# ZechengLi19/CIM

Measured on AMD Instinct MI355X. Metric: images/sec training step (ResNet-50 VOC, ~1k proposals/img) at 1/2/4/8 GPU, higher is better.
Workload: dtype fp32

## Files before the change

### cim_amd/csrc/gemm_pair.hip

```cpp
#include "common.h"
#include <type_traits>
#include "../../include/cim_hip.h"

namespace {

using f32x16 = __attribute__((ext_vector_type(16))) float;
using f16x8 = __attribute__((ext_vector_type(8))) _Float16;
typedef short s16x4 __attribute__((__vector_size__(4 * sizeof(short))));
typedef short s16x8 __attribute__((__vector_size__(8 * sizeof(short))));

#ifndef CIM_PAIR_EXP
#define CIM_PAIR_EXP 0
#endif
static_assert(CIM_PAIR_EXP == 0 || (CIM_PAIR_EXP >= 3 && CIM_PAIR_EXP <= 5), "CIM_PAIR_EXP: 0 (product), 3, 4 or 5");
constexpr bool ABL_NO_LOOP_DMA = CIM_PAIR_EXP == 3 || CIM_PAIR_EXP == 5;
constexpr bool ABL_NO_LOOP_READS = CIM_PAIR_EXP == 4 || CIM_PAIR_EXP == 5;

constexpr int BM = 256, BN = 256, BK = 32;
constexpr int NW = 8, NT = 64 * NW;
constexpr int WNC = 4;
constexpr int WM = 128, WN = BN / WNC, MI = 4, NI = WN / 32;
constexpr int IPW = 32 / NW;
constexpr int OPER = 256 * BK * 4;
constexpr int SLAB = 2 * OPER;
constexpr int LDS_BYTES = 2 * SLAB;
constexpr int RBM = 128, RBK = 16, RNT = 256, RSTAGES = 5;
constexpr int RSTAGE_A = RBM * RBK * 4, RSTAGE_B = BN * RBK * 4, RSTAGE = RSTAGE_A + RSTAGE_B;
constexpr int RIPA = RSTAGE_A / 1024 / 4, RIPB = RSTAGE_B / 1024 / 4;
constexpr int RLDS_BYTES = RSTAGES * RSTAGE;

enum { L_KC = 0, L_MC = 1 };

struct PairArgs {
    const char* A;
    const char* B;
    float* C;
    const float* bias;
    int M, N, K;
    int lda, ldb, ldc;
    int relu;
    int k_per_split;
    long long c_split_stride;
    int batch;
    long long a_bs, b_bs, c_bs;
    const float* a_scale;
    const float* b_scale;
    unsigned* c_amax;
    int tn, tm, tz;
    int tile0;
// ... 235 lines not shown
template <class Loop>
__device__ __forceinline__ void for_valid_subtiles(int rows, Loop&& loop) {
    switch (__builtin_amdgcn_readfirstlane(min(MI, (rows + 31) / 32))) {
        case 1: loop(std::integral_constant<int, 1>{}); break;
        case 2: loop(std::integral_constant<int, 2>{}); break;
        case 3: loop(std::integral_constant<int, 3>{}); break;
        default: loop(std::integral_constant<int, MI>{}); break;
    }
}

template <int MIV>
struct PairFrags {
    f16x8 ah[MIV > 0 ? MIV : 1], al[MIV > 0 ? MIV : 1], bh[NI], bl[NI];
};

template <int MIV>
__device__ __forceinline__ void mma_cluster(f32x16 (&acc)[MI][NI], const f16x8 (&af)[MIV], const f16x8 (&bf)[NI]) {
#pragma unroll
    for (int i = 0; i < MIV; ++i)
#pragma unroll
        for (int j = 0; j < NI; ++j) acc[i][j] = __builtin_amdgcn_mfma_f32_32x32x16_f16(af[i], bf[j], acc[i][j], 0, 0, 0);
}

template <int NMFMA, int NREAD>
__device__ __forceinline__ void interleave_mfma_reads() {
#pragma unroll
    for (int q = 0; q < NMFMA; ++q) {
        __builtin_amdgcn_sched_group_barrier(0x008, 1, 0);
        if (q < NREAD) __builtin_amdgcn_sched_group_barrier(0x100, 1, 0);
    }
    if constexpr (NREAD > NMFMA) __builtin_amdgcn_sched_group_barrier(0x100, NREAD - NMFMA, 0);
    __builtin_amdgcn_sched_barrier(0);
}

template <int TBM, int SLABK>
__device__ __forceinline__ void pair_epilogue(const PairArgs& g, const PairTile<TBM, SLABK>& T, f32x16 (&acc)[MI][NI], float (&bvj)[NI],
                                              int wm, int wn, int lane) {
    const float inv = 1.0f / (g.a_scale[T.zb] * g.b_scale[T.zb]);
#pragma unroll
    for (int j = 0; j < NI; ++j) asm volatile("" : "+v"(bvj[j]));
    float* C = T.C + (size_t)T.zsplit * g.c_split_stride;
    const int m0 = T.m0, n0 = T.n0;
    const int lk = lane >> 5, l31 = lane & 31;
    unsigned amax = 0;
    const bool relu = g.relu != 0;
    if (m0 + TBM <= g.M && n0 + BN <= g.N) {
#pragma unroll
        for (int j = 0; j < NI; ++j) {
            float* cj = C + (size_t)(m0 + wm * WM + 4 * lk) * g.ldc + n0 + wn * WN + j * 32 + l31;
#pragma unroll
            for (int i = 0; i < MI; ++i) {
#pragma unroll
                for (int r = 0; r < 16; ++r) {
                    float v = acc[i][j][r] * inv + bvj[j];
                    if (relu) v = fmaxf(v, 0.0f);
                    amax = max(amax, abs_bits(v));
                    cj[(size_t)(i * 32 + (r & 3) + 8 * (r >> 2)) * g.ldc] = v;
                }
            }
        }
    } else {
#pragma unroll
        for (int j = 0; j < NI; ++j) {
            const int n = n0 + wn * WN + j * 32 + l31;
            if (n >= g.N) continue;
#pragma unroll
            for (int i = 0; i < MI; ++i) {
#pragma unroll
                for (int r = 0; r < 16; ++r) {
                    const int m = m0 + wm * WM + i * 32 + (r & 3) + 8 * (r >> 2) + 4 * lk;
                    if (m >= g.M) continue;
                    float v = acc[i][j][r] * inv + bvj[j];
                    if (relu) v = fmaxf(v, 0.0f);
                    amax = max(amax, abs_bits(v));
                    C[(size_t)m * g.ldc + n] = v;
                }
            }
        }
    }
    if (g.c_amax != nullptr && g.c_split_stride == 0) {
        amax = wave_max_u32(amax);
        if (lane == 0) cim::amax_publish(g.c_amax, amax);
    }
}

template <int AL, int BL, bool ONEP>
__global__ __launch_bounds__(NT, NW / 4) void gemm_pair_kernel(const PairArgs g) {
    extern __shared__ __attribute__((aligned(16))) char smem[];
    const int tid = threadIdx.x;
    const int wave = __builtin_amdgcn_readfirstlane(tid >> 6), lane = tid & 63;
// ... 37 lines not shown
        constexpr std::bool_constant<(MIV > 0 || AL == L_MC)> with_a{};
        PairFrags<MIV> f0, f1;
        auto read = [&](PairFrags<MIV>& f, const char* buf, int ks, auto in_loop) __attribute__((always_inline)) {
            if constexpr (MIV == 0) {
            } else if constexpr (ABL_NO_LOOP_READS && decltype(in_loop)::value) {
                asm volatile("" : "+v"(f.ah[0]), "+v"(f.al[0]), "+v"(f.bh[0]), "+v"(f.bl[0]));
            } else {
#pragma unroll
                for (int j = 0; j < NI; ++j) {
                    f.bh[j] = fb.read(buf + OPER, j, ks, 0);
                    if constexpr (!ONEP) f.bl[j] = fb.read(buf + OPER, j, ks, 1);
                }
#pragma unroll
                for (int i = 0; i < MIV; ++i) {
                    if constexpr (!ONEP) f.al[i] = fa.read(buf, i, ks, 1);
                    f.ah[i] = fa.read(buf, i, ks, 0);
                }
            }
        };
        auto multiply = [&](const PairFrags<MIV>& f) __attribute__((always_inline)) {
            if constexpr (MIV > 0) {
                if constexpr (AL == L_KC && BL == L_KC) __builtin_amdgcn_sched_barrier(0);
                if constexpr (!ONEP) {
                    mma_cluster(acc, f.al, f.bh);
                    mma_cluster(acc, f.ah, f.bl);
                }
                mma_cluster(acc, f.ah, f.bh);
                if constexpr (AL == L_KC && BL == L_KC) __builtin_amdgcn_sched_barrier(0);
            }
        };
        constexpr std::true_type in_loop{};
        read(f0, smem, 0, std::false_type{});
        if constexpr (ABL_NO_LOOP_READS) read(f1, smem, 1, std::false_type{});
        for (int t = 0; t < nslab; ++t) {
            const char* cur = smem + (t & 1) * SLAB;
            const char* nxt = smem + ((t + 1) & 1) * SLAB;
            read(f1, cur, 1, in_loop);
            multiply(f0);
            asm volatile("s_waitcnt vmcnt(0)" ::: "memory");
            __syncthreads();
            if constexpr (!ABL_NO_LOOP_DMA) {
                if (t + 2 < nslab) issue_slab(cur, with_a);
            }
            if (t + 1 < nslab) read(f0, nxt, 0, in_loop);
            multiply(f1);
        }
    };
    if (wm == 1 && T.m0 + WM >= g.M) {
        prologue(std::bool_constant<AL == L_MC>{});
        slab_loop(std::integral_constant<int, 0>{});
        return;
    }
    prologue(std::true_type{});
    for_valid_subtiles(g.M - T.m0 - wm * WM, slab_loop);

    pair_epilogue(g, T, acc, bvj, wm, wn, lane);
}

template <bool ONEP>
__global__ __launch_bounds__(RNT, 2) void gemm_pair_ring_kernel(const PairArgs g) {
    extern __shared__ __attribute__((aligned(16))) char smem[];
    const int tid = threadIdx.x;
    const int wave = __builtin_amdgcn_readfirstlane(tid >> 6), lane = tid & 63;
    const int wn = wave;
    const PairTile<RBM, RBK> T(g);
    const int nslab = T.nslab;
// ... 390 lines not shown
```

### cim_amd/csrc/roi_align.hip

```cpp
#include <cstdlib>
#include "common.h"
#include "wino7_tile.h"
#include "../../include/cim_hip.h"

namespace {

struct RoiGeom {
    float x1, y1, bw, bh, count;
    int gw, gh, b;
};

#pragma clang fp contract(off)
__device__ __forceinline__ RoiGeom roi_geom(const float* __restrict__ roi, float scale, int P, int sampling_ratio,
                                            int aligned) {
    RoiGeom g;
    const float off = aligned ? 0.5f : 0.0f;
    g.b = (int)roi[0];
    g.x1 = roi[1] * scale - off;
    g.y1 = roi[2] * scale - off;
    const float x2 = roi[3] * scale - off;
    const float y2 = roi[4] * scale - off;
    float rw = x2 - g.x1, rh = y2 - g.y1;
    if (!aligned) {
        rw = fmaxf(rw, 1.0f);
// ... 457 lines not shown
        rs_column_walk(s_rows, s_wa, s_wb, nrows, R.ncols, R.xlo, C, R.fb + c, s_wx, al, ah, bl, bh);
        typedef float ga_f4 __attribute__((ext_vector_type(4)));
#pragma unroll
        for (int pw = 0; pw < 7; ++pw) {
            if (pw >= P) break;
            float* dst = out + (((size_t)k * P + ph0) * P + pw) * OC + c;
            __builtin_nontemporal_store(ga_f4{al[pw].x, al[pw].y, ah[pw].x, ah[pw].y}, reinterpret_cast<ga_f4*>(dst));
            if (MASKCAT) {
                const float m = masks[((size_t)k * P + ph0) * P + pw];
                __builtin_nontemporal_store(ga_f4{m * al[pw].x, m * al[pw].y, m * ah[pw].x, m * ah[pw].y}, reinterpret_cast<ga_f4*>(dst + C));
            }
            if (two) {
                float* dst2 = dst + (size_t)P * OC;
                __builtin_nontemporal_store(ga_f4{bl[pw].x, bl[pw].y, bh[pw].x, bh[pw].y}, reinterpret_cast<ga_f4*>(dst2));
                if (MASKCAT) {
                    const float m = masks[((size_t)k * P + ph0 + 1) * P + pw];
                    __builtin_nontemporal_store(ga_f4{m * bl[pw].x, m * bl[pw].y, m * bh[pw].x, m * bh[pw].y}, reinterpret_cast<ga_f4*>(dst2 + C));
                }
            }
        }
    }
}

__global__ __launch_bounds__(256) void roi_align_wino7_pair_kernel(const float* __restrict__ feat, const float* __restrict__ masks,
                                                                   float* __restrict__ V, int C, int H, int W, int K, int Rs,
                                                                   const float* __restrict__ rec_all,
                                                                   const float* __restrict__ scale) {
    constexpr int P = 7;
    __shared__ __attribute__((aligned(16))) float4 s_patch[49 * 64];
    __shared__ __attribute__((aligned(16))) float s_wx[RS_MAXD][8];
    __shared__ float s_wa[4][RS_MAXD], s_wb[4][RS_MAXD];
    __shared__ int s_rows[4][RS_MAXD];
    __shared__ float s_mask[49];
    const int r = blockIdx.x, slice = blockIdx.y, tid = threadIdx.x, lane = tid & 63, wave = tid >> 6;
    const int c = slice * 256 + lane * 4;
    const size_t C2 = 2 * (size_t)C, MC = (size_t)Rs * C2;
    if (r >= K) {
        if (c < C)
            for (int q = wave; q < 121; q += 4) {
                float* dst = V + (size_t)q * MC + (size_t)r * C2 + c;
                __builtin_nontemporal_store(w7_u4{0, 0, 0, 0}, reinterpret_cast<w7_u4*>(dst));
                __builtin_nontemporal_store(w7_u4{0, 0, 0, 0}, reinterpret_cast<w7_u4*>(dst + C));
            }
        return;
    }
    const int k = r;
    const RoiRec R = roi_rec(rec_all, feat, k, C, H, W, P);
    const int ph0 = wave * 2;
    const bool two = ph0 + 1 < P;
    const int nrows = rs_row_list(R, ph0, two, H, W, lane, s_rows[wave], s_wa[wave], s_wb[wave]);
    rs_fill_wx(s_wx, R, P, W, tid, 256);
    if (tid < 49) s_mask[tid] = masks[(size_t)k * 49 + tid];
    __syncthreads();
    if (c < C) {
        ga_f2 al[7], ah[7], bl[7], bh[7];
        rs_column_walk(s_rows[wave], s_wa[wave], s_wb[wave], nrows, R.ncols, R.xlo, C, R.fb + c, s_wx, al, ah, bl, bh);
#pragma unroll
        for (int pw = 0; pw < 7; ++pw) {
            s_patch[(ph0 * P + pw) * 64 + lane] = make_float4(al[pw].x, al[pw].y, ah[pw].x, ah[pw].y);
            if (two) s_patch[((ph0 + 1) * P + pw) * 64 + lane] = make_float4(bl[pw].x, bl[pw].y, bh[pw].x, bh[pw].y);
        }
    }
    __syncthreads();
    if (c >= C) return;
    const size_t off = (size_t)r * C2 + c;
    const auto plain = [&](int iy, int ix) { return s_patch[(iy * P + ix) * 64 + lane]; };
    const auto masked = [&](int iy, int ix) { return vmul(s_mask[iy * P + ix], s_patch[(iy * P + ix) * 64 + lane]); };
// ... 465 lines not shown

extern "C" int cim_roi_align_bwd_ws(const float* grad_out, const float* rois, float* grad_in, int B, int C, int H, int W,
                                    int K, int P, float spatial_scale, int sampling_ratio, int aligned, float* workspace,
                                    int tables_ready, float* scratch, void* stream) {
    return run_bwd<false>(__func__, grad_out, rois, nullptr, grad_in, B, C, H, W, K, P, spatial_scale, sampling_ratio, aligned, workspace,
                          tables_ready, scratch, stream);
}

extern "C" int cim_roi_align_maskcat_bwd(const float* grad_cat, const float* rois, const float* masks, float* grad_in,
                                         int B, int C, int H, int W, int K, int P, float spatial_scale,
                                         int sampling_ratio, int aligned, float* workspace, void* stream) {
    return run_bwd<true>(__func__, grad_cat, rois, masks, grad_in, B, C, H, W, K, P, spatial_scale, sampling_ratio, aligned, workspace,
                         0, nullptr, stream);
}

extern "C" int cim_roi_align_maskcat_bwd_ws(const float* grad_cat, const float* rois, const float* masks, float* grad_in,
                                            int B, int C, int H, int W, int K, int P, float spatial_scale,
                                            int sampling_ratio, int aligned, float* workspace, int tables_ready,
                                            float* scratch, void* stream) {
    return run_bwd<true>(__func__, grad_cat, rois, masks, grad_in, B, C, H, W, K, P, spatial_scale, sampling_ratio, aligned, workspace,
                         tables_ready, scratch, stream);
}
#undef ROI_CHECK_ARG

extern "C" int cim_roi_align_wino7_pair_fwd(const float* feat, const float* rois, const float* masks, void* V, const float* scale,
                                           int B, int C, int H, int W, int K, int Rs, int P, float spatial_scale,
                                           int sampling_ratio, int aligned, float* workspace, void* stream) {
    CIM_CHECK_ARG(feat && rois && masks && V && scale && workspace);
    CIM_CHECK_ARG(B > 0 && C > 0 && C % 8 == 0 && H > 0 && W > 0 && K > 0 && Rs >= K && P == 7);
    CIM_CHECK_ARG(H <= RS_MAXD && W <= RS_MAXD && (long long)H * W * C < (1ll << 30));
    hipStream_t st = cim::as_stream(stream);
    hipLaunchKernelGGL(roi_tables_kernel, dim3(K), dim3(256), sizeof(float) * roi_rec_words(P, H, W), st, rois, workspace, K, P, H, W,
                       spatial_scale, sampling_ratio, aligned);
    hipLaunchKernelGGL(roi_align_wino7_pair_kernel, dim3((unsigned)Rs, (unsigned)((C + 255) / 256)), dim3(256), 0, st, feat, masks,
                       (float*)V, C, H, W, K, Rs, workspace, scale);
    CIM_CHECK_LAUNCH();
    return 0;
}

extern "C" int cim_roi_align_forms(int B, int C, int H, int W, int K, int P, int maskcat, int has_workspace, int tables_ready,
                                   int* fwd_form, int* bwd_form, int* bwd_builds_tables) {
    CIM_CHECK_ARG(B > 0 && C > 0 && H > 0 && W > 0 && K >= 0 && P > 0 && P <= 65535);
    CIM_CHECK_ARG(fwd_form && bwd_form && bwd_builds_tables && (has_workspace || !tables_ready));
    const RoiForms f = roi_forms(B, C, H, W, K, P, maskcat != 0, has_workspace != 0, tables_ready != 0);
    *fwd_form = f.fwd;
    *bwd_form = f.bwd;
    *bwd_builds_tables = f.bwd_builds_tables ? 1 : 0;
    return 0;
}

extern "C" long long cim_roi_align_bwd_workspace(int K, int P, int H, int W) {
    return (long long)sizeof(float) * (long long)K * roi_rec_words(P, H, W);
}

extern "C" long long cim_roi_align_bwd_scratch(int K, int B, int C, int H, int W) {
    const int GS = rg_group_size(K, B, C, H, W);
    const long long groups = (K + GS - 1) / GS;
    return groups > 1 ? (long long)sizeof(float) * groups * B * H * W * C : 0;
}
```

### cim_amd/csrc/winograd.hip

```cpp
#include "common.h"
#include "../../include/cim_hip.h"
#include "wino7_tile.h"

namespace {

__device__ __forceinline__ float4 f4(float v) { return make_float4(v, v, v, v); }
__device__ __forceinline__ void fma2(float2& a, float s, float2 v) { a.x = fmaf(s, v.x, a.x); a.y = fmaf(s, v.y, a.y); }

typedef float w7_v2 __attribute__((ext_vector_type(2)));
typedef float w7_v4 __attribute__((ext_vector_type(4)));

constexpr int W7_VOUT = 4;
constexpr int W7_VDX = 2;
constexpr int W7_VMF = 1;
constexpr int W7_MF_WAVES = 1;
constexpr int W7_FB_WAVES = 3;
constexpr int W7_WG_CI = 4;

template <int N> struct w7_vec;
template <> struct w7_vec<1> { typedef float T; };
template <> struct w7_vec<2> { typedef float2 T; };
template <> struct w7_vec<4> { typedef float4 T; };
__device__ __forceinline__ void w7_store(float* p, float v) { __builtin_nontemporal_store(v, p); }
__device__ __forceinline__ void w7_store(float* p, float2 v) { __builtin_nontemporal_store(w7_v2{v.x, v.y}, reinterpret_cast<w7_v2*>(p)); }
__device__ __forceinline__ void w7_store(float* p, float4 v) {
    __builtin_nontemporal_store(w7_v4{v.x, v.y, v.z, v.w}, reinterpret_cast<w7_v4*>(p));
}
__device__ __forceinline__ void vzero(float& a) { a = 0.0f; }
__device__ __forceinline__ void vzero(float2& a) { a = make_float2(0.f, 0.f); }
__device__ __forceinline__ void vzero(float4& a) { a = make_float4(0.f, 0.f, 0.f, 0.f); }
__device__ __forceinline__ void vfma(float& a, float s, float v) { a = fmaf(s, v, a); }
__device__ __forceinline__ void vfma(float2& a, float s, float2 v) { fma2(a, s, v); }
__device__ __forceinline__ void vfma(float4& a, float s, float4 v) { fma4(a, s, v); }
__device__ __forceinline__ float vamax(float4 v) { return fmaxf(fmaxf(fabsf(v.x), fabsf(v.y)), fmaxf(fabsf(v.z), fabsf(v.w))); }
__device__ __forceinline__ void vrelu(float4& v) { v = make_float4(fmaxf(v.x, 0.f), fmaxf(v.y, 0.f), fmaxf(v.z, 0.f), fmaxf(v.w, 0.f)); }
template <typename T> __device__ __forceinline__ T vload(const float* p) { return *reinterpret_cast<const T*>(p); }
template <typename T> __device__ __forceinline__ T vload_once(const float* p) {
    if constexpr (sizeof(T) == 4) return __builtin_nontemporal_load(p);
    else if constexpr (sizeof(T) == 8) { const w7_v2 v = __builtin_nontemporal_load(reinterpret_cast<const w7_v2*>(p)); return make_float2(v.x, v.y); }
    else { const w7_v4 v = __builtin_nontemporal_load(reinterpret_cast<const w7_v4*>(p)); return make_float4(v.x, v.y, v.z, v.w); }
}

__device__ __forceinline__ void w7_zero_rows(float* __restrict__ V, int q0, int nq, int r, int Rs, int C) {
    for (int q = q0; q < q0 + nq; ++q)
        for (int c = threadIdx.x * 4; c < C; c += 1024)
            *reinterpret_cast<float4*>(V + ((size_t)q * Rs + r) * C + c) = make_float4(0.f, 0.f, 0.f, 0.f);
}

__global__ __launch_bounds__(256) void wino7_input_pair_kernel(const float* __restrict__ x, float* __restrict__ V, int R, int Rs,
// ... 153 lines not shown
        for (int c = threadIdx.x * 4; c < C; c += 256 * 4) {
            float4 d[OA][OB];
#pragma unroll
            for (int a = 0; a < OA; ++a)
#pragma unroll
                for (int b = 0; b < OB; ++b)
                    d[a][b] = vload<float4>(dy + (((size_t)r * 7 + W7::OUT0[KA] + a) * 7 + W7::OUT0[KB] + b) * C + c);
            w7_dy_tile_regs<KA, KB, ADJ>(d, D, (size_t)Rs * C, (size_t)r * C + c, scale);
        }
    });
}

constexpr int W7_FB_LDW = 260;

template <int KA, int KB, bool ADJ>
__device__ __forceinline__ void w7_fb_tile(const float* __restrict__ s, int lane, float* __restrict__ img, size_t MC, size_t rc,
                                           const float* __restrict__ scale) {
    constexpr int OA = W7::OUT[KA], OB = W7::OUT[KB];
    float4 d[OA][OB];
#pragma unroll
    for (int a = 0; a < OA; ++a)
#pragma unroll
        for (int b = 0; b < OB; ++b)
            d[a][b] = *reinterpret_cast<const float4*>(s + ((W7::OUT0[KA] + a) * 7 + W7::OUT0[KB] + b) * W7_FB_LDW + 4 * lane);
    if (img != nullptr) w7_dy_tile_regs<KA, KB, ADJ>(d, img, MC, rc, scale);
}

__global__ __launch_bounds__(256, W7_FB_WAVES) void wino7_flatten_bwd_dy_pair_kernel(const float* __restrict__ dX, const float* __restrict__ y,
                                                                        float* __restrict__ E, float* __restrict__ D,
                                                                        float* __restrict__ bsum, int R, int Rs, int C,
                                                                        const float* __restrict__ sE, const float* __restrict__ sD) {
    __shared__ __attribute__((aligned(16))) float s[49 * W7_FB_LDW];
    __shared__ float4 red[3][64];
    const int r = blockIdx.x, c0 = blockIdx.y * 256, tid = threadIdx.x, lane = tid & 63;
    const int w = __builtin_amdgcn_readfirstlane(tid >> 6);
    const size_t MC = (size_t)Rs * C, rc = (size_t)r * C + c0 + 4 * lane;
    if (r >= R) {
        const w7_u4 z = {0u, 0u, 0u, 0u};
        for (int q = w; q < 121; q += 4) {
            if (E != nullptr) __builtin_nontemporal_store(z, reinterpret_cast<w7_u4*>(E + (size_t)q * MC + rc));
            if (D != nullptr) __builtin_nontemporal_store(z, reinterpret_cast<w7_u4*>(D + (size_t)q * MC + rc));
        }
        return;
    }
    const float4* __restrict__ src4 = reinterpret_cast<const float4*>(dX + ((size_t)r * C + c0) * 49);
    for (int i = tid; i < 49 * 64; i += 256) {
        const float4 v = vload_once<float4>(reinterpret_cast<const float*>(src4 + i));
        int c = (4 * i) / 49, p = 4 * i - 49 * c;
        const float e[4] = {v.x, v.y, v.z, v.w};
#pragma unroll
        for (int k = 0; k < 4; ++k) {
            s[p * W7_FB_LDW + c] = e[k];
            if (++p == 49) { p = 0; ++c; }
        }
    }
    __syncthreads();
    float4 part = f4(0.f);
    for (int p = w; p < 49; p += 4) {
        float4* sp = reinterpret_cast<float4*>(s + p * W7_FB_LDW + 4 * lane);
        float4 d = *sp;
        if (y != nullptr) {
            const float4 yv = *reinterpret_cast<const float4*>(y + ((size_t)r * 49 + p) * C + c0 + 4 * lane);
            d.x = yv.x > 0.0f ? d.x : 0.0f;
            d.y = yv.y > 0.0f ? d.y : 0.0f;
            d.z = yv.z > 0.0f ? d.z : 0.0f;
            d.w = yv.w > 0.0f ? d.w : 0.0f;
            *sp = d;
        }
        part.x += d.x; part.y += d.y; part.z += d.z; part.w += d.w;
    }
    if (bsum != nullptr && w > 0) red[w - 1][lane] = part;
    __syncthreads();
    if (bsum != nullptr && w == 0) {
        const float4 a = part, b = red[0][lane], c = red[1][lane], e = red[2][lane];
        *reinterpret_cast<float4*>(bsum + rc) = make_float4((a.x + b.x) + (c.x + e.x), (a.y + b.y) + (c.y + e.y),
                                                            (a.z + b.z) + (c.z + e.z), (a.w + b.w) + (c.w + e.w));
    }
    w7_for_tile(w, [&](auto t) __attribute__((always_inline)) {
        w7_fb_tile<t.KA, t.KB, true>(s, lane, E, MC, rc, sE);
        w7_fb_tile<1 - t.KA, 1 - t.KB, false>(s, lane, D, MC, rc, sD);
    });
}

__global__ void wino7_pair_scales_kernel(const unsigned* __restrict__ amax, int n_amax, const unsigned* __restrict__ amax_mul, int kind,
                                         float* __restrict__ scale) {
    const int q = threadIdx.x;
    if (q >= 121) return;
    unsigned mbits = 0;
    for (int t = 0; t < n_amax; ++t) mbits = max(mbits, amax[t] & 0x7fffffffu);
    float dmax = __uint_as_float(mbits);
    if (amax_mul != nullptr) dmax *= fmaxf(1.0f, __uint_as_float(amax_mul[0] & 0x7fffffffu));
    const int type = q < 36 ? 0 : q < 66 ? 1 : q < 96 ? 2 : 3;
    const int ka = type >> 1, kb = type & 1, nb = kb ? 5 : 6, pl = q - W7::QOFF[type];
    const int pi = pl / nb, pj = pl % nb;
    float fa = 0.0f, fb = 0.0f;
    if (kind == 0) {
        for (int t = 0; t < 6; ++t) { fa += fabsf(W7_BT[ka][pi][t]); fb += fabsf(W7_BT[kb][pj][t]); }
    } else if (kind == 1) {
        for (int t = 0; t < 3; ++t) { fa += fabsf(W7_G[ka][pi][t]); fb += fabsf(W7_G[kb][pj][t]); }
    } else if (kind == 2) {
        for (int t = 0; t < 4; ++t) { fa += fabsf(W7_GD[ka][pi][t]); fb += fabsf(W7_GD[kb][pj][t]); }
    } else {
// ... 24 lines not shown
        }
#pragma unroll
        for (int l = 0; l < NB; ++l) {
            const int xx = W7::IN0[KB] + l;
            if (xx < 0 || xx >= P) continue;
#pragma unroll
            for (int j = 0; j < NB; ++j)
                if (W7_BT[KB][j][l] != 0.0f) vfma(acc[yy][xx], W7_BT[KB][j][l], t[j]);
        }
    }
}

__global__ __launch_bounds__(256) void wino7_dx_kernel(const float* __restrict__ M, float* __restrict__ dx, int R, int C) {
    constexpr int VW = W7_VDX;
    typedef typename w7_vec<VW>::T VT;
    const int r = blockIdx.x;
    const size_t MC = (size_t)R * C;
    for (int c = (blockIdx.y * 256 + threadIdx.x) * VW; c < C; c += gridDim.y * 256 * VW) {
        VT acc[7][7];
#pragma unroll
        for (int y = 0; y < 7; ++y)
#pragma unroll
            for (int x = 0; x < 7; ++x) vzero(acc[y][x]);
        const size_t rc = (size_t)r * C + c;
        w7_for_all_tiles([&](auto t) __attribute__((always_inline)) { w7_dx_tile<t.KA, t.KB, VT>(M, MC, rc, acc); });
#pragma unroll
        for (int y = 0; y < 7; ++y)
#pragma unroll
            for (int x = 0; x < 7; ++x) w7_store(dx + (((size_t)r * 7 + y) * 7 + x) * C + c, acc[y][x]);
    }
}

__global__ __launch_bounds__(256, W7_MF_WAVES) void wino7_dx_maskfold_kernel(const float* __restrict__ M, const float* __restrict__ masks,
                                                                float* __restrict__ dbox, int R, int Cb) {
    constexpr int VW = W7_VMF;
    typedef typename w7_vec<VW>::T VT;
    const int r = blockIdx.x;
    const size_t C2 = 2 * (size_t)Cb, MC = (size_t)R * C2;
    const float* __restrict__ mk = masks + (size_t)r * 49;
    for (int c = (blockIdx.y * 256 + threadIdx.x) * VW; c < Cb; c += gridDim.y * 256 * VW) {
        VT acc[7][7];
#pragma unroll
        for (int y = 0; y < 7; ++y)
#pragma unroll
            for (int x = 0; x < 7; ++x) vzero(acc[y][x]);
        const size_t rc = (size_t)r * C2 + c;
        w7_for_all_tiles([&](auto t) __attribute__((always_inline)) { w7_dx_tile<t.KA, t.KB, VT>(M, MC, rc + Cb, acc); });
#pragma unroll
        for (int y = 0; y < 7; ++y)
#pragma unroll
            for (int x = 0; x < 7; ++x) {
                const float m = mk[y * 7 + x];
                VT z;
                vzero(z);
                vfma(z, m, acc[y][x]);
                acc[y][x] = z;
            }
        w7_for_all_tiles([&](auto t) __attribute__((always_inline)) { w7_dx_tile<t.KA, t.KB, VT>(M, MC, rc, acc); });
#pragma unroll
        for (int y = 0; y < 7; ++y)
#pragma unroll
            for (int x = 0; x < 7; ++x) w7_store(dbox + (((size_t)r * 7 + y) * 7 + x) * Cb + c, acc[y][x]);
    }
}

template <int KA, int KB, typename VT>
__device__ __forceinline__ void w7_wgrad_tile(const float* __restrict__ dU, size_t KN, size_t idx, VT (&acc)[3][3]) {
    constexpr int NA = W7::NP[KA], NB = W7::NP[KB], Q0 = W7::QOFF[KA * 2 + KB];
    VT s[3][NB];
#pragma unroll
    for (int a = 0; a < 3; ++a)
#pragma unroll
        for (int j = 0; j < NB; ++j) vzero(s[a][j]);
// ... 57 lines not shown
        const int row = e / ROW, col = e - row * ROW;
        dW[((size_t)(co0 + row) * Cin + ci0) * 9 + col] = t[row][col];
    }
}

__global__ __launch_bounds__(256) void flatten_chw_bwd_kernel(const float* __restrict__ src, const float* __restrict__ y,
                                                              float* __restrict__ dst, int PP, int C, float* __restrict__ bsum) {
    __shared__ float t[64][65];
    const int r = blockIdx.x, c0 = blockIdx.y * 64, tid = threadIdx.x;
    const size_t base = (size_t)r * PP * C;
    for (int e = tid; e < PP * 64; e += 256) {
        const int c = e / PP, p = e - c * PP;
        t[p][c] = src[base + (size_t)c0 * PP + e];
    }
    __syncthreads();
    float part = 0.0f;
    for (int e = tid; e < PP * 64; e += 256) {
        const int p = e >> 6, c = e & 63;
        const size_t o = base + (size_t)p * C + c0 + c;
        const float v = (y == nullptr || y[o] > 0.0f) ? t[p][c] : 0.0f;
        dst[o] = v;
        part += v;
    }
    if (bsum != nullptr) {
        __syncthreads();
        t[tid >> 6][tid & 63] = part;
        __syncthreads();
        if (tid < 64) bsum[(size_t)r * C + c0 + tid] = (t[0][tid] + t[1][tid]) + (t[2][tid] + t[3][tid]);
    }
}

__global__ __launch_bounds__(256) void flatten_chw_pair_kernel(const float* __restrict__ src, float* __restrict__ dst, int R,
                                                               int PP, int C, const float* __restrict__ scale) {
    __shared__ float t[64][65];
    const int r = blockIdx.x, c0 = blockIdx.y * 64, tid = threadIdx.x;
    float* out = dst + (size_t)r * PP * C + (size_t)c0 * PP;
    const int chunks = PP * 8;
    if (r >= R) {
        for (int q = tid; q < chunks * 2; q += 256) *reinterpret_cast<float4*>(out + q * 4) = make_float4(0.f, 0.f, 0.f, 0.f);
        return;
    }
    const size_t base = (size_t)r * PP * C;
    for (int e = tid; e < PP * 64; e += 256) {
        const int p = e >> 6, c = e & 63;
        t[p][c] = src[base + (size_t)p * C + c0 + c];
    }
    __syncthreads();
    const float s = scale[0];
    for (int q = tid; q < chunks; q += 256) {
        float v[8];
#pragma unroll
        for (int k = 0; k < 8; ++k) {
            const int e = q * 8 + k, c = e / PP, p = e - c * PP;
            v[k] = t[p][c] * s;
        }
        unsigned hh[4], ll[4];
#pragma unroll
        for (int e = 0; e < 4; ++e) cim::pair_split2(v[2 * e], v[2 * e + 1], hh[e], ll[e]);
        const w7_u4 h = {hh[0], hh[1], hh[2], hh[3]}, l = {ll[0], ll[1], ll[2], ll[3]};
        *reinterpret_cast<w7_u4*>(out + q * 8) = h;
        *reinterpret_cast<w7_u4*>(out + q * 8 + 4) = l;
    }
}

}

extern "C" int cim_wino_wgrad_output(const float* dU, float* dW, int Cout, int Cin, int tile, void* stream) {
    CIM_CHECK_ARG(dU && dW && Cout > 0 && Cin > 0);
    CIM_CHECK_ARG(tile == 7);
    const size_t n = (size_t)Cout * Cin;
    if (Cout % 64 == 0 && Cin % W7_WG_CI == 0 && Cin / W7_WG_CI <= 65535)
        hipLaunchKernelGGL(wino7_wgrad_out_rows_kernel, dim3(Cout / 64, Cin / W7_WG_CI), dim3(64 * W7_WG_CI), 0, cim::as_stream(stream), dU,
                           dW, Cout, Cin);
    else hipLaunchKernelGGL(wino7_wgrad_out_kernel, dim3((unsigned)((n + 255) / 256)), dim3(256), 0, cim::as_stream(stream), dU, dW, Cout, Cin);
    CIM_CHECK_LAUNCH();
    return 0;
}

extern "C" int cim_wino_dx_adjoint_output(const float* M, float* dx, int R, int P, int C, int tile, void* stream) {
    CIM_CHECK_ARG(R > 0 && P > 0 && P <= 64 && C > 0 && C % 4 == 0);
    CIM_CHECK_ARG(M && dx && tile == 7 && P == 7 && R <= 2147483647);
    int chunks = (C + 256 * W7_VDX - 1) / (256 * W7_VDX);
    if (chunks > 4) chunks = 4;
    hipLaunchKernelGGL(wino7_dx_kernel, dim3(R, chunks), dim3(256), 0, cim::as_stream(stream), M, dx, R, C);
    CIM_CHECK_LAUNCH();
    return 0;
}

extern "C" int cim_wino7_dx_maskfold(const float* M, const float* masks, float* dbox, int R, int Cb, void* stream) {
    CIM_CHECK_ARG(M && masks && dbox && R > 0 && Cb > 0 && Cb % 4 == 0);
    int chunks = (Cb + 256 * W7_VMF - 1) / (256 * W7_VMF);
    if (chunks > 4) chunks = 4;
    hipLaunchKernelGGL(wino7_dx_maskfold_kernel, dim3(R, chunks), dim3(256), 0, cim::as_stream(stream), M, masks, dbox, R, Cb);
    CIM_CHECK_LAUNCH();
    return 0;
}

extern "C" int cim_wino7_pair_scales(const uint32_t* amax, int n_amax, const uint32_t* amax_mul, int kind, float* scale, void* stream) {
    CIM_CHECK_ARG(amax && scale && kind >= 0 && kind <= 3 && n_amax >= 1 && n_amax <= 65536);
    hipLaunchKernelGGL(wino7_pair_scales_kernel, dim3(1), dim3(128), 0, cim::as_stream(stream), amax, n_amax, amax_mul, kind, scale);
    CIM_CHECK_LAUNCH();
    return 0;
}

extern "C" int cim_wino7_input_pair(const float* x, void* V, const float* scale, int R, int Rs, int C, void* stream) {
    CIM_CHECK_ARG(x && V && scale && R > 0 && Rs >= R && C > 0 && C % 8 == 0);
    hipLaunchKernelGGL(wino7_input_pair_kernel, dim3(Rs, 4), dim3(256), 0, cim::as_stream(stream), x, (float*)V, R, Rs, C, scale);
    CIM_CHECK_LAUNCH();
    return 0;
}

extern "C" int cim_wino7_filter_pair(const float* W, void* U, const float* scale, int Cout, int Cin, void* stream) {
    CIM_CHECK_ARG(W && U && scale && Cout > 0 && Cin > 0 && Cin % 8 == 0);
    const size_t n = (size_t)Cout * Cin;
    hipLaunchKernelGGL(wino7_filter_pair_kernel, dim3((unsigned)((n + 255) / 256)), dim3(256), 0, cim::as_stream(stream), W,
                       (float*)U, Cout, Cin, scale);
    CIM_CHECK_LAUNCH();
    return 0;
}

extern "C" int cim_wino7_dy_pair(const float* dy, void* D, const float* scale, int R, int Rs, int C, int adjoint, void* stream) {
    CIM_CHECK_ARG(dy && D && scale && R > 0 && Rs >= R && C > 0 && C % 8 == 0);
    if (adjoint) hipLaunchKernelGGL(wino7_dy_pair_kernel<true>, dim3(Rs, 4), dim3(256), 0, cim::as_stream(stream), dy, (float*)D, R, Rs, C, scale);
    else hipLaunchKernelGGL(wino7_dy_pair_kernel<false>, dim3(Rs, 4), dim3(256), 0, cim::as_stream(stream), dy, (float*)D, R, Rs, C, scale);
    CIM_CHECK_LAUNCH();
    return 0;
}

extern "C" int cim_wino7_flatten_bwd_dy_pair(const float* dX, const float* relu_y, void* E, const float* scale_e, void* D,
                                             const float* scale_d, float* bias_partial, int R, int Rs, int C, void* stream) {
    CIM_CHECK_ARG(dX && (E || D) && (!E || scale_e) && (!D || scale_d) && R > 0 && Rs >= R && C > 0 && C % 256 == 0 && C / 256 <= 65535);
    hipLaunchKernelGGL(wino7_flatten_bwd_dy_pair_kernel, dim3(Rs, C / 256), dim3(256), 0, cim::as_stream(stream), dX, relu_y, (float*)E,
                       (float*)D, bias_partial, R, Rs, C, scale_e, scale_d);
    CIM_CHECK_LAUNCH();
    return 0;
}

extern "C" int cim_wino7_output_amax(const float* M, const float* bias, float* y, int R, int C, int relu, uint32_t* y_amax,
                                     void* stream) {
    CIM_CHECK_ARG(M && y && R > 0 && C > 0 && C % 4 == 0);
    hipLaunchKernelGGL(wino7_output_kernel, dim3(R, 4), dim3(256), 0, cim::as_stream(stream), M, bias, y, R, C, relu, y_amax);
    CIM_CHECK_LAUNCH();
    return 0;
}

extern "C" int cim_flatten_chw_pair(const float* src, void* dst, const float* scale, int R, int Rs, int PP, int C, void* stream) {
    CIM_CHECK_ARG(src && dst && scale && R > 0 && Rs >= R && PP > 0 && PP <= 64 && C > 0 && C % 64 == 0 && C / 64 <= 65535);
    hipLaunchKernelGGL(flatten_chw_pair_kernel, dim3(Rs, C / 64), dim3(256), 0, cim::as_stream(stream), src, (float*)dst, R, PP, C, scale);
    CIM_CHECK_LAUNCH();
    return 0;
}

extern "C" int cim_flatten_chw_bwd_bias(const float* src, const float* relu_y, float* dst, float* bias_partial, int R, int PP,
                                        int C, void* stream) {
    CIM_CHECK_ARG(src && dst && R > 0 && PP > 0 && PP <= 64 && C > 0 && C % 64 == 0 && C / 64 <= 65535);
    hipLaunchKernelGGL(flatten_chw_bwd_kernel, dim3(R, C / 64), dim3(256), 0, cim::as_stream(stream), src, relu_y, dst, PP, C, bias_partial);
    CIM_CHECK_LAUNCH();
    return 0;
}
```

Baseline: 76.13.

## Interleave LDS reads and split DMA issue across MFMA clusters for KC/MC pair GEMM

Adds a specialized slab loop for the A-K-contiguous / B-M-contiguous three-product pair GEMM that places LDS fragment reads between MFMAs (two reads per MFMA) using sched_group_barrier. It splits the next-slab global-to-LDS DMA issue of A and B between the MFMA clusters so memory issue overlaps with matrix math. It also adds an ablation flag that skips epilogue stores. The ablation is off by default. The new schedule pins instruction order and may raise register pressure or stall if reads are not ready.

```diff
diff --git a/cim_amd/csrc/gemm_pair.hip b/cim_amd/csrc/gemm_pair.hip
--- a/cim_amd/csrc/gemm_pair.hip
+++ b/cim_amd/csrc/gemm_pair.hip
@@ -12,9 +12,10 @@
 #ifndef CIM_PAIR_EXP
 #define CIM_PAIR_EXP 0
 #endif
-static_assert(CIM_PAIR_EXP == 0 || (CIM_PAIR_EXP >= 3 && CIM_PAIR_EXP <= 5), "CIM_PAIR_EXP: 0 (product), 3, 4 or 5");
+static_assert(CIM_PAIR_EXP == 0 || (CIM_PAIR_EXP >= 3 && CIM_PAIR_EXP <= 6), "CIM_PAIR_EXP: 0 (product), 3, 4, 5 or 6");
 constexpr bool ABL_NO_LOOP_DMA = CIM_PAIR_EXP == 3 || CIM_PAIR_EXP == 5;
 constexpr bool ABL_NO_LOOP_READS = CIM_PAIR_EXP == 4 || CIM_PAIR_EXP == 5;
+constexpr bool ABL_NO_STORES = CIM_PAIR_EXP == 6;
 
 constexpr int BM = 256, BN = 256, BK = 32;
 constexpr int NW = 8, NT = 64 * NW;
@@ -316,6 +317,17 @@
     if constexpr (NREAD > NMFMA) __builtin_amdgcn_sched_group_barrier(0x100, NREAD - NMFMA, 0);
     __builtin_amdgcn_sched_barrier(0);
 }
+template <int NMFMA, int NREAD, int PER>
+__device__ __forceinline__ void interleave_mfma_reads_by() {
+#pragma unroll
+    for (int q = 0; q < NMFMA; ++q) {
+        __builtin_amdgcn_sched_group_barrier(0x008, 1, 0);
+        if ((q + 1) * PER <= NREAD) __builtin_amdgcn_sched_group_barrier(0x100, PER, 0);
+    }
+    constexpr int PLACED = (NREAD / PER < NMFMA ? NREAD / PER : NMFMA) * PER;
+    if constexpr (NREAD > PLACED) __builtin_amdgcn_sched_group_barrier(0x100, NREAD - PLACED, 0);
+    __builtin_amdgcn_sched_barrier(0);
+}
 
 template <int TBM, int SLABK>
 __device__ __forceinline__ void pair_epilogue(const PairArgs& g, const PairTile<TBM, SLABK>& T, f32x16 (&acc)[MI][NI], float (&bvj)[NI],
@@ -339,7 +351,7 @@
                     float v = acc[i][j][r] * inv + bvj[j];
                     if (relu) v = fmaxf(v, 0.0f);
                     amax = max(amax, abs_bits(v));
-                    cj[(size_t)(i * 32 + (r & 3) + 8 * (r >> 2)) * g.ldc] = v;
+                    if (!ABL_NO_STORES || v == 123456.75f) cj[(size_t)(i * 32 + (r & 3) + 8 * (r >> 2)) * g.ldc] = v;
                 }
             }
         }
@@ -443,6 +455,41 @@
         constexpr std::true_type in_loop{};
         read(f0, smem, 0, std::false_type{});
         if constexpr (ABL_NO_LOOP_READS) read(f1, smem, 1, std::false_type{});
+        if constexpr (AL == L_KC && BL == L_MC && MIV > 0 && !ONEP) {
+            constexpr int NR = 4 * NI + 2 * MIV, NM = MIV * NI;
+            auto step = [&](PairFrags<MIV>& nf, const char* nbuf, int nks, const PairFrags<MIV>& f, auto dma_a, auto dma_b) __attribute__((always_inline)) {
+                __builtin_amdgcn_sched_barrier(0);
+                read(nf, nbuf, nks, in_loop);
+                mma_cluster(acc, f.al, f.bh);
+                interleave_mfma_reads_by<NM, NR, 2>();
+                dma_a();
+                __builtin_amdgcn_sched_barrier(0);
+                mma_cluster(acc, f.ah, f.bl);
+                __builtin_amdgcn_sched_barrier(0);
+                dma_b();
+                __builtin_amdgcn_sched_barrier(0);
+                mma_cluster(acc, f.ah, f.bh);
+                __builtin_amdgcn_sched_barrier(0);
+            };
+            auto none = [] {};
+            for (int t = 0; t < nslab; ++t) {
+                const char* cur = smem + (t & 1) * SLAB;
+                const char* nxt = smem + ((t + 1) & 1) * SLAB;
+                step(f1, cur, 1, f0, none, none);
+                asm volatile("s_waitcnt vmcnt(0)" ::: "memory");
+                __syncthreads();
+                const bool more = !ABL_NO_LOOP_DMA && t + 2 < nslab;
+                step(f0, nxt, 0, f1, [&]() __attribute__((always_inline)) { if (more) sa.issue(ak, cur, wave); },
+                     [&]() __attribute__((always_inline)) {
+                         if (more) {
+                             sb.issue(bk, cur + OPER, wave);
+                             ak += a_adv;
+                             bk += b_adv;
+                         }
+                     });
+            }
+            return;
+        }
         for (int t = 0; t < nslab; ++t) {
             const char* cur = smem + (t & 1) * SLAB;
             const char* nxt = smem + ((t + 1) & 1) * SLAB;
```

Result: no change. 76.46 (median of 2 runs) (+0.4%).

## Flatten grids to 1D and batch loads in wino7 flatten/pair kernels

Applied to the files above, without the earlier changes.

Several kernels (roi_align wino7 pair, flatten_bwd_dy_pair, dx_maskfold, flatten_chw_pair) switch from a 2D grid to a 1D grid, so ROI and channel slice are decoded from blockIdx.x and neighbouring blocks share a ROI. flatten_bwd_dy_pair now issues all dX and relu_y loads up front into registers before the LDS transpose, which raises memory-level parallelism at the cost of more registers. flatten_chw_pair is rewritten with 128-channel chunks, dynamic shared memory, batched float4 loads and a shared pair-store helper. The added register arrays may lower occupancy, and the new flatten kernel assumes C divisible by 32 per chunk.

```diff
diff --git a/cim_amd/csrc/roi_align.hip b/cim_amd/csrc/roi_align.hip
--- a/cim_amd/csrc/roi_align.hip
+++ b/cim_amd/csrc/roi_align.hip
@@ -513,7 +513,8 @@
     __shared__ float s_wa[4][RS_MAXD], s_wb[4][RS_MAXD];
     __shared__ int s_rows[4][RS_MAXD];
     __shared__ float s_mask[49];
-    const int r = blockIdx.x, slice = blockIdx.y, tid = threadIdx.x, lane = tid & 63, wave = tid >> 6;
+    const int nsl = (C + 255) / 256, r = blockIdx.x / nsl, slice = blockIdx.x - r * nsl;
+    const int tid = threadIdx.x, lane = tid & 63, wave = tid >> 6;
     const int c = slice * 256 + lane * 4;
     const size_t C2 = 2 * (size_t)C, MC = (size_t)Rs * C2;
     if (r >= K) {
@@ -1045,7 +1046,7 @@
     hipStream_t st = cim::as_stream(stream);
     hipLaunchKernelGGL(roi_tables_kernel, dim3(K), dim3(256), sizeof(float) * roi_rec_words(P, H, W), st, rois, workspace, K, P, H, W,
                        spatial_scale, sampling_ratio, aligned);
-    hipLaunchKernelGGL(roi_align_wino7_pair_kernel, dim3((unsigned)Rs, (unsigned)((C + 255) / 256)), dim3(256), 0, st, feat, masks,
+    hipLaunchKernelGGL(roi_align_wino7_pair_kernel, dim3((unsigned)((size_t)Rs * ((C + 255) / 256))), dim3(256), 0, st, feat, masks,
                        (float*)V, C, H, W, K, Rs, workspace, scale);
     CIM_CHECK_LAUNCH();
     return 0;
diff --git a/cim_amd/csrc/winograd.hip b/cim_amd/csrc/winograd.hip
--- a/cim_amd/csrc/winograd.hip
+++ b/cim_amd/csrc/winograd.hip
@@ -15,6 +15,8 @@
 constexpr int W7_VMF = 1;
 constexpr int W7_MF_WAVES = 1;
 constexpr int W7_FB_WAVES = 3;
+constexpr int W7_FF_CH = 128;
+constexpr int W7_FF_LOADS = 7;
 constexpr int W7_WG_CI = 4;
 
 template <int N> struct w7_vec;
@@ -234,7 +236,7 @@
                                                                         const float* __restrict__ sE, const float* __restrict__ sD) {
     __shared__ __attribute__((aligned(16))) float s[49 * W7_FB_LDW];
     __shared__ float4 red[3][64];
-    const int r = blockIdx.x, c0 = blockIdx.y * 256, tid = threadIdx.x, lane = tid & 63;
+    const int nsl = C / 256, r = blockIdx.x / nsl, c0 = (blockIdx.x - r * nsl) * 256, tid = threadIdx.x, lane = tid & 63;
     const int w = __builtin_amdgcn_readfirstlane(tid >> 6);
     const size_t MC = (size_t)Rs * C, rc = (size_t)r * C + c0 + 4 * lane;
     if (r >= R) {
@@ -245,31 +247,56 @@
         }
         return;
     }
+    constexpr int NL = (49 * 64 + 255) / 256, NY = 13;
     const float4* __restrict__ src4 = reinterpret_cast<const float4*>(dX + ((size_t)r * C + c0) * 49);
-    for (int i = tid; i < 49 * 64; i += 256) {
-        const float4 v = vload_once<float4>(reinterpret_cast<const float*>(src4 + i));
-        int c = (4 * i) / 49, p = 4 * i - 49 * c;
-        const float e[4] = {v.x, v.y, v.z, v.w};
-#pragma unroll
-        for (int k = 0; k < 4; ++k) {
-            s[p * W7_FB_LDW + c] = e[k];
-            if (++p == 49) { p = 0; ++c; }
-        }
+    float4 v[NL], yv[NY];
+#pragma unroll
+    for (int u = 0; u < NL; ++u) {
+        const int i = tid + u * 256;
+        if (i < 49 * 64) v[u] = vload_once<float4>(reinterpret_cast<const float*>(src4 + i));
+    }
+    if (y != nullptr) {
+#pragma unroll
+        for (int u = 0; u < NY; ++u) {
+            const int p = w + 4 * u;
+            if (p < 49) yv[u] = *reinterpret_cast<const float4*>(y + ((size_t)r * 49 + p) * C + c0 + 4 * lane);
+        }
+    }
+#pragma unroll
+    for (int u = 0; u < NL; ++u) {
+        const int i = tid + u * 256;
+        if (i < 49 * 64) {
+            int c = (4 * i) / 49, p = 4 * i - 49 * c;
+            const float e[4] = {v[u].x, v[u].y, v[u].z, v[u].w};
+#pragma unroll
+            for (int k = 0; k < 4; ++k) {
+                s[p * W7_FB_LDW + c] = e[k];
+                if (++p == 49) { p = 0; ++c; }
+            }
+        }
+    }
+    if (y != nullptr) {
+#pragma unroll
+        for (int u = 0; u < NY; ++u)
+            if (w + 4 * u < 49) asm volatile("" : "+v"(yv[u].x), "+v"(yv[u].y), "+v"(yv[u].z), "+v"(yv[u].w));
     }
     __syncthreads();
     float4 part = f4(0.f);
-    for (int p = w; p < 49; p += 4) {
-        float4* sp = reinterpret_cast<float4*>(s + p * W7_FB_LDW + 4 * lane);
-        float4 d = *sp;
-        if (y != nullptr) {
-            const float4 yv = *reinterpret_cast<const float4*>(y + ((size_t)r * 49 + p) * C + c0 + 4 * lane);
-            d.x = yv.x > 0.0f ? d.x : 0.0f;
-            d.y = yv.y > 0.0f ? d.y : 0.0f;
-            d.z = yv.z > 0.0f ? d.z : 0.0f;
-            d.w = yv.w > 0.0f ? d.w : 0.0f;
-            *sp = d;
-        }
-        part.x += d.x; part.y += d.y; part.z += d.z; part.w += d.w;
+#pragma unroll
+    for (int u = 0; u < NY; ++u) {
+        const int p = w + 4 * u;
+        if (p < 49) {
+            float4* sp = reinterpret_cast<float4*>(s + p * W7_FB_LDW + 4 * lane);
+            float4 d = *sp;
+            if (y != nullptr) {
+                d.x = yv[u].x > 0.0f ? d.x : 0.0f;
+                d.y = yv[u].y > 0.0f ? d.y : 0.0f;
+                d.z = yv[u].z > 0.0f ? d.z : 0.0f;
+                d.w = yv[u].w > 0.0f ? d.w : 0.0f;
+                *sp = d;
+            }
+            part.x += d.x; part.y += d.y; part.z += d.z; part.w += d.w;
+        }
     }
     if (bsum != nullptr && w > 0) red[w - 1][lane] = part;
     __syncthreads();
@@ -360,13 +387,13 @@
 }
 
 __global__ __launch_bounds__(256, W7_MF_WAVES) void wino7_dx_maskfold_kernel(const float* __restrict__ M, const float* __restrict__ masks,
-                                                                float* __restrict__ dbox, int R, int Cb) {
+                                                                float* __restrict__ dbox, int R, int Cb, int nchunk) {
     constexpr int VW = W7_VMF;
     typedef typename w7_vec<VW>::T VT;
-    const int r = blockIdx.x;
+    const int r = blockIdx.x / nchunk, chunk = blockIdx.x - r * nchunk;
     const size_t C2 = 2 * (size_t)Cb, MC = (size_t)R * C2;
     const float* __restrict__ mk = masks + (size_t)r * 49;
-    for (int c = (blockIdx.y * 256 + threadIdx.x) * VW; c < Cb; c += gridDim.y * 256 * VW) {
+    for (int c = (chunk * 256 + threadIdx.x) * VW; c < Cb; c += nchunk * 256 * VW) {
         VT acc[7][7];
 #pragma unroll
         for (int y = 0; y < 7; ++y)
@@ -490,35 +517,38 @@
 
 __global__ __launch_bounds__(256) void flatten_chw_pair_kernel(const float* __restrict__ src, float* __restrict__ dst, int R,
                                                                int PP, int C, const float* __restrict__ scale) {
-    __shared__ float t[64][65];
-    const int r = blockIdx.x, c0 = blockIdx.y * 64, tid = threadIdx.x;
+    extern __shared__ __attribute__((aligned(16))) float ff_t[];
+    const int nsl = (C + W7_FF_CH - 1) / W7_FF_CH, r = blockIdx.x / nsl, c0 = (blockIdx.x - r * nsl) * W7_FF_CH;
+    const int tid = threadIdx.x, lane = tid & 63;
+    const int w = __builtin_amdgcn_readfirstlane(tid >> 6);
+    const int nch = min(W7_FF_CH, C - c0), nq = nch * PP / 4;
     float* out = dst + (size_t)r * PP * C + (size_t)c0 * PP;
-    const int chunks = PP * 8;
     if (r >= R) {
-        for (int q = tid; q < chunks * 2; q += 256) *reinterpret_cast<float4*>(out + q * 4) = make_float4(0.f, 0.f, 0.f, 0.f);
+        for (int q = tid; q < nq; q += 256) w7_store(out + q * 4, f4(0.f));
         return;
     }
-    const size_t base = (size_t)r * PP * C;
-    for (int e = tid; e < PP * 64; e += 256) {
-        const int p = e >> 6, c = e & 63;
-        t[p][c] = src[base + (size_t)p * C + c0 + c];
+    const float* in = src + (size_t)r * PP * C + c0;
+    const int ngb = nch / 32, nit = ((PP + 7) / 8) * ngb;
+    const int dp = lane >> 3, dg = lane & 7;
+    for (int it0 = w; it0 < nit; it0 += 4 * W7_FF_LOADS) {
+        float4 v[W7_FF_LOADS];
+#pragma unroll
+        for (int u = 0; u < W7_FF_LOADS; ++u) {
+            const int it = it0 + 4 * u, pb = it / ngb, g = (it - pb * ngb) * 8 + dg, p = pb * 8 + dp;
+            if (it < nit && p < PP) v[u] = vload<float4>(in + (size_t)p * C + 4 * g);
+        }
+#pragma unroll
+        for (int u = 0; u < W7_FF_LOADS; ++u) {
+            const int it = it0 + 4 * u, pb = it / ngb, g = (it - pb * ngb) * 8 + dg, p = pb * 8 + dp;
+            if (it < nit && p < PP) {
+                float* tp = ff_t + 4 * g * PP + p;
+                tp[0] = v[u].x; tp[PP] = v[u].y; tp[2 * PP] = v[u].z; tp[3 * PP] = v[u].w;
+            }
+        }
     }
     __syncthreads();
     const float s = scale[0];
-    for (int q = tid; q < chunks; q += 256) {
-        float v[8];
-#pragma unroll
-        for (int k = 0; k < 8; ++k) {
-            const int e = q * 8 + k, c = e / PP, p = e - c * PP;
-            v[k] = t[p][c] * s;
-        }
-        unsigned hh[4], ll[4];
-#pragma unroll
-        for (int e = 0; e < 4; ++e) cim::pair_split2(v[2 * e], v[2 * e + 1], hh[e], ll[e]);
-        const w7_u4 h = {hh[0], hh[1], hh[2], hh[3]}, l = {ll[0], ll[1], ll[2], ll[3]};
-        *reinterpret_cast<w7_u4*>(out + q * 8) = h;
-        *reinterpret_cast<w7_u4*>(out + q * 8 + 4) = l;
-    }
+    for (int q = tid; q < nq; q += 256) w7_store_pair(out + q * 4, *reinterpret_cast<const float4*>(ff_t + q * 4), s);
 }
 
 }
@@ -549,7 +579,8 @@
     CIM_CHECK_ARG(M && masks && dbox && R > 0 && Cb > 0 && Cb % 4 == 0);
     int chunks = (Cb + 256 * W7_VMF - 1) / (256 * W7_VMF);
     if (chunks > 4) chunks = 4;
-    hipLaunchKernelGGL(wino7_dx_maskfold_kernel, dim3(R, chunks), dim3(256), 0, cim::as_stream(stream), M, masks, dbox, R, Cb);
+    hipLaunchKernelGGL(wino7_dx_maskfold_kernel, dim3((unsigned)((size_t)R * chunks)), dim3(256), 0, cim::as_stream(stream), M, masks, dbox,
+                       R, Cb, chunks);
     CIM_CHECK_LAUNCH();
     return 0;
 }
@@ -588,7 +619,7 @@
 extern "C" int cim_wino7_flatten_bwd_dy_pair(const float* dX, const float* relu_y, void* E, const float* scale_e, void* D,
                                              const float* scale_d, float* bias_partial, int R, int Rs, int C, void* stream) {
     CIM_CHECK_ARG(dX && (E || D) && (!E || scale_e) && (!D || scale_d) && R > 0 && Rs >= R && C > 0 && C % 256 == 0 && C / 256 <= 65535);
-    hipLaunchKernelGGL(wino7_flatten_bwd_dy_pair_kernel, dim3(Rs, C / 256), dim3(256), 0, cim::as_stream(stream), dX, relu_y, (float*)E,
+    hipLaunchKernelGGL(wino7_flatten_bwd_dy_pair_kernel, dim3((unsigned)((size_t)Rs * (C / 256))), dim3(256), 0, cim::as_stream(stream), dX, relu_y, (float*)E,
                        (float*)D, bias_partial, R, Rs, C, scale_e, scale_d);
     CIM_CHECK_LAUNCH();
     return 0;
@@ -604,7 +635,8 @@
 
 extern "C" int cim_flatten_chw_pair(const float* src, void* dst, const float* scale, int R, int Rs, int PP, int C, void* stream) {
     CIM_CHECK_ARG(src && dst && scale && R > 0 && Rs >= R && PP > 0 && PP <= 64 && C > 0 && C % 64 == 0 && C / 64 <= 65535);
-    hipLaunchKernelGGL(flatten_chw_pair_kernel, dim3(Rs, C / 64), dim3(256), 0, cim::as_stream(stream), src, (float*)dst, R, PP, C, scale);
+    hipLaunchKernelGGL(flatten_chw_pair_kernel, dim3((unsigned)((size_t)Rs * ((C + W7_FF_CH - 1) / W7_FF_CH))), dim3(256), sizeof(float) * W7_FF_CH * PP,
+                       cim::as_stream(stream), src, (float*)dst, R, PP, C, scale);
     CIM_CHECK_LAUNCH();
     return 0;
 }
```

Result: no change. 77.71 before, 78.36 after, median of 3 (+0.8%).
